# stefavpolito/EEPACC_MPC_CasADi_MATLAB

Hardware: AMD Instinct MI355X
Metric: QP steps/sec (whole node), ABMPC N=30 dense QP at batch 4096 (higher is better)
Workload: dtype f64; 1 GPU; ABMPC N=30 fp64, batch=4096 synthetic S2 ego/lead scenarios per GPU, closed loop; batch_per_gpu=4096, horizon=30, steps_per_launch=2252, parallelism=instances sharded across 1 GPU(s), no data-path collective

## Files before the change

eepacc_mpc_casadi_matlab_amd/csrc/eepacc_ab_impl.inc:

```
namespace eepacc {
namespace EEPACC_IMPL_NS {
using namespace wv;

constexpr bool kMoveBlocking = EEPACC_IMPL_MB;
constexpr bool kBaseline = EEPACC_IMPL_BL;
constexpr bool kIce = EEPACC_IMPL_ICE;
constexpr bool kTargetVeh = EEPACC_IMPL_TV;
static_assert(!kTargetVeh || kBaseline, "the target-vehicle MPC is a variant of the baseline controller");


#undef PTIC
#undef PTOC
#undef RTOC
#ifdef EEPACC_AB_TIMING
__device__ unsigned long long g_ab_prof[24];
#define PTIC(L) long long _pt = wall_clock64()
#define PTOC(L, slot) do { long long _n = wall_clock64(); (L).prof[slot] += _n - _pt; _pt = _n; } while (0)
#else
#define PTIC(L)
#define PTOC(L, slot)
#endif

constexpr double kInf = 1e300;
constexpr double kTolViol = 1e-11;
// ... 47 lines not shown

struct Lane {
    int lane, N;
    double T, tau, tau1;
    double tau_rev;
    double ba[kNumRowTypes];
    unsigned valid;
#ifdef EEPACC_AB_TIMING
    long long prof[24];
#endif
    unsigned ign;
    unsigned long long kmask;
    double lbF, lbS, lbV, lbH;
    unsigned long long code;
    double chw;
    double g0;
    double a, sh, vh, am1;
    int base;
};

__device__ __forceinline__ int code_of(const Lane& L, int t) { return (int)((L.code >> (4 * t)) & 15ull); }
__device__ __forceinline__ void set_code(Lane& L, int t, int c) {
    L.code = (L.code & ~(15ull << (4 * t))) | ((unsigned long long)c << (4 * t));
}

struct Cfg {
    int N;
    double tau_min, wF, wS, wV, wH, qH;
    int mb_len;
    const int32_t *mb_lead, *mb_end;
};

__device__ __forceinline__ double mb_reduce(const Lane& L, const Cfg& c, double x) {
    if constexpr (!kMoveBlocking) return x;
    if (c.mb_len == 0) return x;
    const int k = L.lane <= L.N ? L.lane : L.N;
    const int end = c.mb_end[k];
    const bool leader = c.mb_lead[k] == k && L.lane < L.N;
    double acc = x;
    for (int d = 1; d < c.mb_len; ++d) {
        const double y = __shfl_down(x, d, 64);
        if (L.lane + d <= end) acc += y;
    }
    return leader ? acc : 0.0;
}
__device__ __forceinline__ double mb_expand(const Lane& L, const Cfg& c, double x) {
    if constexpr (!kMoveBlocking) return x;
    if (c.mb_len == 0) return x;
    const int k = L.lane < L.N ? L.lane : 0;
    const double y = __shfl(x, c.mb_lead[k], 64);
    return L.lane < L.N ? y : x;
}

__device__ __forceinline__ double group_w(const Cfg& c, int g) {
    return g == G_F ? c.wF : (g == G_S ? c.wS : (g == G_V ? c.wV : c.wH));
}
__device__ __forceinline__ double group_lb(const Lane& L, int g) {
    return g == G_F ? L.lbF : (g == G_S ? L.lbS : (g == G_V ? L.lbV : L.lbH));
}
__device__ __forceinline__ int lane_group(const Lane& L, int t) { return L.lane == L.N ? G_NONE : group_of(t); }

__device__ __forceinline__ double row_val(const Lane& L, const Cfg& c, int t, double ba_t) {
    return row_al(t) * L.sh + row_be(t, c.tau_min, L.chw) * L.vh + row_ga(t) * L.a + row_de(t, L.lane) * L.am1 - ba_t;
}

constexpr unsigned long long kNib = 0x1111111111111111ull;
__device__ __forceinline__ unsigned long long codes_eq1(unsigned long long c) { return c & ~(c >> 1) & kNib; }
__device__ __forceinline__ unsigned long long codes_eq2(unsigned long long c) { return (c >> 1) & ~c & kNib; }
__device__ __forceinline__ constexpr unsigned long long type_range(int t0, int t1) {
    return ((t1 >= 15 ? ~0ull : ((1ull << (4 * (t1 + 1))) - 1ull)) & ~((1ull << (4 * t0)) - 1ull)) & kNib;
}
__device__ __forceinline__ int rows_below(const Lane& L, int t) {
    return __popcll(codes_eq1(L.code) & ((1ull << (4 * t)) - 1ull));
}
__device__ __forceinline__ int pivot_of(const Lane& L, int g) {
    const unsigned long long rng = kBaseline ? (g == G_F ? type_range(R_AMAX, R_VINC) : 0ull)
                                             : (g == G_F ? type_range(R_AMAX, R_VCURV)
                                                         : (g == G_S ? type_range(R_SAFE1, R_VTL) : (g == G_V ? type_range(R_VINC, R_VINC) : 0ull)));
    const unsigned long long two = codes_eq2(L.code) & rng;
    return two ? ((__ffsll((long long)two) - 1) >> 2) : -1;
}

__device__ __forceinline__ void hom_traj(const Lane& L, double x, double& sh, double& vh) {
    double xi = (L.lane < L.N) ? x : 0.0;
    vh = scan_excl(L.T * xi);
    double inc = (L.lane < L.N) ? (L.T * vh + 0.5 * L.T * L.T * xi) : 0.0;
    sh = scan_excl(inc);
}

template <int NS> constexpr bool kPackedHe = NS > 32;
template <int NS> constexpr int kHeDoubles = kPackedHe<NS> ? NS * (NS + 1) / 2 : NS * NS;

__device__ __forceinline__ double normal_at(const Lane& L, int kq, double al, double be, double ga, double de, double tau_kq) {
    double c = 0.0;
    const int j = L.lane;
    if (j < L.N) {
        if (j < kq) c = L.T * (be + al * (0.5 * L.T + tau_kq - L.tau1));
        if (j == kq) c += ga;
        if (j == kq - 1) c += de;
    }
    return c;
}

template <int NS>
__device__ __forceinline__ double adjoint(const Lane& L, const double* ws, const double* wv, const double* wa, double* tmp) {
    const int r = L.lane, N = L.N;
    const int k = N - r;
    const bool in = k >= 0;
    const double s = in ? ws[k] : 0.0, v = in ? wv[k] : 0.0;
    const double tk = in ? L.tau_rev : 0.0;
    const double WS = scan_excl(s), WV = scan_excl(v), WST = scan_excl(s * tk);
    if (in) { tmp[k] = WS; tmp[(NS + 1) + k] = WV; tmp[2 * (NS + 1) + k] = WST; }
    WSYNC();
    const int j = L.lane;
    double g = 0.0;
    if (j < N) g = wa[j] + L.T * (tmp[(NS + 1) + j] + tmp[2 * (NS + 1) + j] - (L.tau1 - 0.5 * L.T) * tmp[j]);
    WSYNC();
    return g;
}

enum Ev : int { EV_NONE = 0, EV_DROP, EV_COMPL, EV_DROPH, EV_CAP, EV_CAPIN };

template <int MMAX, int NS>
__device__ __forceinline__ void he_rank1(const Lane& L, const Cfg& c, WaveMem<MMAX, NS>& M, double* He,
                                         const double* tauv, int k, bool add) {
    const int lane = L.lane, N = L.N;
    const double chwk = bcast(L.chw, k);
    const double nk = mb_reduce(L, c, normal_at(L, k, 1.0, chwk, 0.0, 0.0, tauv[k]));
    if (lane < NS) M.yv[lane] = nk;
    WSYNC();
    const double y = he_mul<NS, kPackedHe<NS>>(He, M.yv, N, lane);
    double sy, vy;
    hom_traj(L, mb_expand(L, c, y), sy, vy);
    const double ny = bcast(sy + chwk * vy, k);
    const double kappa = add ? c.qH / (1.0 + c.qH * ny) : -c.qH / (1.0 - c.qH * ny);
    if (lane < NS) M.ub[lane] = y;
    WSYNC();
    if (lane < NS) he_sub_outer<NS, kPackedHe<NS>>(He, M.ub, kappa * y, lane);
    WSYNC();
}

template <int MMAX, int NS>
__device__ __forceinline__ void he_sync(Lane& L, const Cfg& c, WaveMem<MMAX, NS>& M, double* He, const double* tauv) {
    if constexpr (!row_live(R_HWP)) return;
    const unsigned long long want = __ballot(L.lane < L.N && code_of(L, R_HWP) == 3);
    unsigned long long diff = want ^ L.kmask;
    while (diff) {
        const int k = __ffsll((long long)diff) - 1;
        diff &= diff - 1;
        he_rank1(L, c, M, He, tauv, k, ((want >> k) & 1ull) != 0ull);
    }
    L.kmask = want;
}

template <int NS>
__device__ __forceinline__ void he_load_base(double* He, const double* __restrict__ base, int N, int lane) {
    if constexpr (kPackedHe<NS>) {
        if (lane < NS)
            for (int i = lane; i < NS; ++i) He[he_tri(i) + lane] = (i < N && lane < N) ? base[i * N + lane] : 0.0;
    } else {
#pragma unroll 4
        for (int e = lane; e < NS * NS; e += 64) {
            const int i = e / NS, j = e % NS;
            He[e] = (i < N && j < N) ? base[i * N + j] : 0.0;
        }
    }
}

template <int MMAX, int NS>
__device__ __forceinline__ int rebuild_and_factor(Lane& L, const Cfg& c, WaveMem<MMAX, NS>& M, double* Hs, const double* tauv,
                                                  const FastInfo& F) {
    const int lane = L.lane, N = L.N;
#undef RTOC
#ifdef EEPACC_AB_TIMING
    long long _q = wall_clock64();
#define RTOC(slot) do { long long _n = wall_clock64(); L.prof[slot] += _n - _q; _q = _n; } while (0)
#else
#define RTOC(slot)
#endif
    he_sync(L, c, M, Hs, tauv);
    RTOC(9);
    const int cnt = __popcll(codes_eq1(L.code));
    double basef = scan_excl((double)cnt);
    L.base = (int)(basef + 0.5);
    int m = (int)(wave_sum((double)cnt) + 0.5);
    if (m > schur_capacity<MMAX>()) return -2;
    struct PRow { double al, be, ga, de, d; };
    PRow PR[3];
#pragma unroll
    for (int gi = 0; gi < 3; ++gi) {
        const int g = G_F + gi;
        const int p = pivot_of(L, g);
        PRow r{0.0, 0.0, 0.0, 0.0, -group_lb(L, g)};
        if (p >= 0) {
            double pba = 0.0;
#pragma unroll
            for (int u = R_AMAX; u <= R_VINC; ++u) if (row_live(u) && u == p) pba = L.ba[u];
            r.al = row_al(p); r.be = row_be(p, c.tau_min, L.chw); r.ga = row_ga(p); r.de = row_de(p, lane); r.d = pba;
        }
        PR[gi] = r;
    }
    int pos = L.base;
#pragma unroll
    for (int t = 0; t < kNumRowTypes; ++t) {
        if (!row_live(t)) continue;
        int cd = code_of(L, t);
        if (cd == 1) {
            int g = lane_group(L, t);
            double al = row_al(t), be = row_be(t, c.tau_min, L.chw), ga = row_ga(t), de = row_de(t, lane);
            double d = L.ba[t];
            if (g == G_H) {
                d += L.lbH;
            } else if (g != G_NONE) {
                const int gi = group_of(t) - G_F;
                if (gi >= 0 && gi < 3) { const PRow& r = PR[gi]; al -= r.al; be -= r.be; ga -= r.ga; de -= r.de; d -= r.d; }
            }
            M.e_al[pos] = al; M.e_be[pos] = be; M.e_ga[pos] = ga; M.e_de[pos] = de;
            M.e_d[pos] = d; M.w_k[pos] = lane;
            ++pos;
        }
    }
    WSYNC();
    RTOC(10);
    if (m == 0) return 0;
    const unsigned short* rc = rc_table<MMAX>();
    if (F.fast == 1 && m == F.m_old + 1 && F.m_old > 0) {
        const int pl = rows_below(L, F.tq);
        const int p = __builtin_amdgcn_readlane(L.base + pl, __builtin_amdgcn_readfirstlane(F.kq));
        schur_insert(M.P, M.rv, rc, m, p, 1.0 / F.zz, lane);
        RTOC(12);
        return m;
    }
    if (F.fast == 2 && m == F.m_old - 1) {
        schur_remove(M.P, M.ws, rc, F.m_old, m, F.drop_pos, lane);
        RTOC(12);
        return m;
    }
    {
        const int ki = lane < m ? M.w_k[lane] : 0;
        const int kim1 = ki > 0 ? ki - 1 : 0;
        const double eal = lane < m ? M.e_al[lane] : 0.0, ebe = lane < m ? M.e_be[lane] : 0.0;
        const double ega = (lane < m && ki < N) ? M.e_ga[lane] : 0.0;
        const double ede = (lane < m && ki > 0 && ki <= N) ? M.e_de[lane] : 0.0;
        for (int j = 0; j < m; j += 2) {
            const bool two = j + 1 < m;
            const int j1 = two ? j + 1 : j;
            const int kj0 = M.w_k[j], kj1 = M.w_k[j1];
            const double c0 = mb_reduce(L, c, normal_at(L, kj0, M.e_al[j], M.e_be[j], M.e_ga[j], M.e_de[j], tauv[kj0]));
            const double c1 = mb_reduce(L, c, normal_at(L, kj1, M.e_al[j1], M.e_be[j1], M.e_ga[j1], M.e_de[j1], tauv[kj1]));
            if (lane < NS) { M.yv[lane] = c0; M.lam[lane] = c1; }
            WSYNC();
            double u0, u1;
            he_mul2<NS, kPackedHe<NS>>(Hs, M.yv, M.lam, N, lane, u0, u1);
            u0 = mb_expand(L, c, u0); u1 = mb_expand(L, c, u1);
            WSYNC();
            double su0, vu0, su1, vu1;
            hom_traj(L, u0, su0, vu0);
            hom_traj(L, u1, su1, vu1);
            const double sx = eal * __shfl(su0, ki, 64) + ebe * __shfl(vu0, ki, 64) + ega * __shfl(u0, ki, 64) + ede * __shfl(u0, kim1, 64);
            const double sy = eal * __shfl(su1, ki, 64) + ebe * __shfl(vu1, ki, 64) + ega * __shfl(u1, ki, 64) + ede * __shfl(u1, kim1, 64);
            if (lane >= j && lane < m) M.P[pidx(lane, j)] = sx;
            if (two && lane >= j + 1 && lane < m) M.P[pidx(lane, j + 1)] = sy;
        }
        WSYNC();
    }
    RTOC(11);
    const int singular = schur_invert(M.P, M.sv, M.ws, rc, m, lane);
    RTOC(12);
    if (singular) return kBaseline ? -(9 + singular) : -1;
    return m;
}

template <int MMAX, int NS>
__device__ __forceinline__ double gradient_side(const Lane& L, const Cfg& c, WaveMem<MMAX, NS>& M, int m, bool with_lam,
                                double lam_q, int kq, double qal, double qbe, double qga, double qde) {
    const int lane = L.lane, N = L.N;
    double s = 0.0, v = 0.0, a0 = 0.0, a1 = 0.0;
    if (lane < N) {
#pragma unroll
        for (int t = R_AMAX; t <= R_VINC; ++t) {
            if (row_live(t) && code_of(L, t) == 2) {
                double w = group_w(c, group_of(t));
                s += w * row_al(t); v += w * row_be(t, c.tau_min, L.chw);
                a0 += w * row_ga(t); a1 += w * row_de(t, lane);
            }
        }
    }
    if (lane < N && EEPACC_HWP_ON(L)) {
        const double wl = c.wH - c.qH * L.ba[R_HWP];
        s += wl * row_al(R_HWP); v += wl * row_be(R_HWP, c.tau_min, L.chw);
    }
// ... 7 lines not shown
        atomicAdd(&M.wv[ki], l * M.e_be[lane]);
        if (ki < N && M.e_ga[lane] != 0.0) atomicAdd(&M.wa[ki], l * M.e_ga[lane]);
        if (ki > 0 && M.e_de[lane] != 0.0) atomicAdd(&M.wa[ki - 1], l * M.e_de[lane]);
    }
    if (lam_q != 0.0 && lane == 0) {
        atomicAdd(&M.ws[kq], lam_q * qal);
        atomicAdd(&M.wv[kq], lam_q * qbe);
        if (kq < N && qga != 0.0) atomicAdd(&M.wa[kq], lam_q * qga);
        if (kq > 0 && qde != 0.0) atomicAdd(&M.wa[kq - 1], lam_q * qde);
    }
    WSYNC();
    double g = adjoint<NS>(L, M.ws, M.wv, M.wa, M.ub);
    return (lane < N) ? g + L.g0 : 0.0;
}

template <int MMAX, int NS>
__device__ __forceinline__ double direction_side(const Lane& L, WaveMem<MMAX, NS>& M, int m, int kq,
                                                 double qal, double qbe, double qga, double qde) {
    const int lane = L.lane, N = L.N;
    if (lane <= N) { M.ws[lane] = 0.0; M.wv[lane] = 0.0; M.wa[lane] = 0.0; }
    WSYNC();
    if (lane < m) {
        const int ki = M.w_k[lane];
        const double l = -M.rv[lane];
        atomicAdd(&M.ws[ki], l * M.e_al[lane]);
        atomicAdd(&M.wv[ki], l * M.e_be[lane]);
        if (ki < N && M.e_ga[lane] != 0.0) atomicAdd(&M.wa[ki], l * M.e_ga[lane]);
        if (ki > 0 && M.e_de[lane] != 0.0) atomicAdd(&M.wa[ki - 1], l * M.e_de[lane]);
    }
    if (lane == 0) {
        atomicAdd(&M.ws[kq], qal);
        atomicAdd(&M.wv[kq], qbe);
        if (kq < N && qga != 0.0) atomicAdd(&M.wa[kq], qga);
        if (kq > 0 && qde != 0.0) atomicAdd(&M.wa[kq - 1], qde);
    }
    WSYNC();
    return adjoint<NS>(L, M.ws, M.wv, M.wa, M.ub);
}

template <int MMAX, int NS>
__device__ __forceinline__ double rows_dot(const WaveMem<MMAX, NS>& M, int i, int N) {
    return rows_dot_img(M, i, N, M.ub, M.sub, M.vub);
}

template <int MMAX, int NS>
__device__ __forceinline__ void primal_from_multipliers(Lane& L, const Cfg& c, WaveMem<MMAX, NS>& M, const double* Hs, int m,
                                        double lam_q, int kq, double qal, double qbe, double qga, double qde,
                                        double& grad_total) {
    double g = gradient_side(L, c, M, m, true, lam_q, kq, qal, qbe, qga, qde);
    grad_total = g;
    g = mb_reduce(L, c, g);
    if (L.lane < NS) M.yv[L.lane] = g;
    WSYNC();
    L.a = -mb_expand(L, c, he_mul<NS, kPackedHe<NS>>(Hs, M.yv, L.N, L.lane));
    hom_traj(L, L.a, L.sh, L.vh);
    L.am1 = dpp_zero<0x138, 0xf>(L.a);
    if (L.lane < L.N) M.av[L.lane] = L.a;
    if (L.lane <= L.N) { M.shv[L.lane] = L.sh; M.vhv[L.lane] = L.vh; }
    WSYNC();
}

template <int MMAX, int NS>
__device__ __forceinline__ double refine_primal(Lane& L, const Cfg& c, WaveMem<MMAX, NS>& M, const double* Hs, int m,
                                                double lam_q, int kq, double qal, double qbe, double qga, double qde,
                                                double& grad_total, int max_rounds, double res_tol) {
    primal_from_multipliers(L, c, M, Hs, m, lam_q, kq, qal, qbe, qga, qde, grad_total);
    if (m == 0) return 0.0;
    double rel0 = 0.0;
    for (int round = 0; round < max_rounds; ++round) {
        double res = 0.0, rel = 0.0;
        if (L.lane < m) {
            res = rows_dot_img(M, L.lane, L.N, M.av, M.shv, M.vhv) - M.e_d[L.lane];
            rel = fabs(res) / (1.0 + fabs(M.e_d[L.lane]));
            M.sv[L.lane] = res;
        }
        int dummy = L.lane;
        wave_argmax(rel, dummy);
        if (round == 0) rel0 = rel;
        if (!(rel > res_tol)) break;
        WSYNC();
        if (L.lane < m) {
            double acc = 0.0;
            for (int j = 0; j < m; ++j) acc = fma(M.P[pidx(L.lane, j)], M.sv[j], acc);
            M.lam[L.lane] += acc;
        }
        WSYNC();
        primal_from_multipliers(L, c, M, Hs, m, lam_q, kq, qal, qbe, qga, qde, grad_total);
    }
    return rel0;
}

__device__ __forceinline__ double group_xi(const Lane& L, const Cfg& c, int g) {
    int p = pivot_of(L, g);
    if (p < 0) return group_lb(L, g);
    double pba = 0.0;
#pragma unroll
    for (int u = R_AMAX; u <= R_VINC; ++u) if (row_live(u) && u == p) pba = L.ba[u];
    return row_val(L, c, p, pba);
}

template <int MMAX, int NS>
__device__ __forceinline__ int warm_repair(Lane& L, const Cfg& c, const WaveMem<MMAX, NS>& M, int m, bool single, int& drop_pos) {
    const int lane = L.lane, N = L.N;
    double lmax = 0.0;
    if (lane < m) lmax = fabs(M.lam[lane]);
    lmax = wave_max(lmax);
    const double tol = kTolDual * (1.0 + lmax);
// ... 216 lines not shown
        if (F.fast == 0) L.prof[14 + why] += 1;
#endif
        if (F.fast == 0) fast_run = 0;
        const bool inc = inc_next && F.fast != 0;
        inc_next = false;
        F.m_old = m;
        m = rebuild_and_factor(L, c, M, Hs, tauv, F);
        F.fast = 0;
        PTOC(L, 0);
        if constexpr (kBaseline) {
            if (m <= -10 && warm && dep_drops < 8) {
                const int p = -m - 10;
                const int pl = M.w_k[p];
                if (lane == pl) {
                    int idx = p - L.base;
#pragma unroll
                    for (int t = 0; t < kNumRowTypes; ++t) if (row_live(t) && code_of(L, t) == 1) { if (idx == 0) set_code(L, t, 0); --idx; }
                }
                ++dep_drops;
                WSYNC();
                continue;
            }
        }
        if (m < 0) {
#ifdef EEPACC_BL_TRACE
            if (lane == 0 && (gridDim.x == 1 || g_trace_on)) printf("   factor failed (m %d, warm %d)\n", m, (int)warm);
#endif
            if (!warm) { st.status = 2; break; }
            L.code = 0ull;
            he_load_base<NS>(Hs, Hbase, N, lane);
            L.kmask = 0ull;
            WSYNC();
            warm = false;
            continue;
        }
        if (have_q) incoming_row(L, c, q);
        bool scratch = !inc;
        double rel0 = 0.0;
        if (inc && m > 0) {
            double rel = 0.0;
            if (lane < m) rel = fabs(rows_dot_img(M, lane, N, M.av, M.shv, M.vhv) - M.e_d[lane]) / (1.0 + fabs(M.e_d[lane]));
            int dummy = lane;
            wave_argmax(rel, dummy);
            rel0 = rel;
            if (rel0 > 1e-11) { scratch = true; carry_ok = false; }
#ifdef EEPACC_AB_TIMING
            L.prof[23] += scratch ? 1000 : 1;
#endif
        }
        if (scratch && m > 0) {
            double g = mb_reduce(L, c, gradient_side(L, c, M, 0, false, lam_q, q.kq, q.al, q.be, q.ga, q.de));
            if (lane < NS) M.yv[lane] = g;
            WSYNC();
            double h = mb_expand(L, c, he_mul<NS, kPackedHe<NS>>(Hs, M.yv, N, lane));
            double shh, vhh;
            hom_traj(L, h, shh, vhh);
            if (lane < N) M.ub[lane] = h;
            if (lane <= N) { M.sub[lane] = shh; M.vub[lane] = vhh; }
            WSYNC();
            solve_multipliers(M, m, lane, N);
        }
        PTOC(L, 1);
        if (scratch) {
            const double r0 = refine_primal(L, c, M, Hs, m, lam_q, q.kq, q.al, q.be, q.ga, q.de, grad_total, 3, 1e-11);
            if (r0 > rel0) rel0 = r0;
        }
        if (fast_run > 0 && rel0 > 1e-10) p_stale = true;
        PTOC(L, 2);
        if (warm && !have_q) {
            if (m > 0) {
                bool take = false;
                if constexpr (kPfAdds > 0 && !kBaseline) {
                    if (pf_left > 0) {
                        const double lam_l = (lane < m) ? M.lam[lane] : 0.0;
                        const double labs = wave_max(fabs(lam_l)), lneg = wave_max(-lam_l);
                        if (lneg > kTolDual * (1.0 + labs) && lneg <= 0.3 * labs) {
                            const int bpw = find_violation(L, c, 1e-6, best);
                            if (bpw >= 0 && (bpw & 31) < 16) {
                                q.kq = bpw >> 5; q.qcode = bpw & 31; q.is_bound = false; q.tq = q.qcode;
                                q.gq = (q.kq == N) ? G_NONE : group_of(q.qcode);
                                have_q = true; lam_q = 0.0; pf = true; take = true;
                                --pf_left; ++st.iters;
                                incoming_row(L, c, q);
#ifdef EEPACC_BL_TRACE
                                if (lane == 0 && (gridDim.x == 1 || g_trace_on)) printf("   primal first: (%d,%d) viol %.3e, worst multiplier %.3e of %.3e, m %d\n", q.kq, q.qcode, best, -lneg, labs, m);
#endif
                            }
                        }
                    }
                }
                if (!take) {
                const int rep = warm_repair(L, c, M, m, pass < kSinglePasses, F.drop_pos);
#ifdef EEPACC_BL_TRACE
                if (lane == 0 && (gridDim.x == 1 || g_trace_on)) printf("   repair pass %d: m %d -> change %d\n", pass, m, rep);
#endif
                PTOC(L, 3);
                if (rep == 2) F.fast = 2;
                WHY(1);
                if (rep) {
                    if (++pass >= kSinglePasses + 6) {
                        L.code &= ~codes_eq1(L.code);
                        he_load_base<NS>(Hs, Hbase, N, lane);
                        L.kmask = 0ull;
                        WSYNC();
                        warm = false;
                    }
                    continue;
                }
                }
            }
            if (!have_q) warm = false;
        }
        if (!have_q) {
            const int relax_every = 3 * N + 30;
            const double tolv = kTolViol * (st.iters < relax_every ? 1.0 : (st.iters < 2 * relax_every ? 10.0 : (st.iters < 3 * relax_every ? 100.0 : 1000.0)));
            int bp = find_violation(L, c, tolv > tol_floor ? tolv : tol_floor, best);
            if constexpr (kBaseline) {
                if (bp >= 0) {
                    bool again = false;
#pragma unroll
                    for (int h = 0; h < kHist; ++h) again = again || (bp == hist_bp[h] && fabs(best - hist_best[h]) <= 1e-3 * best);
                    if (again) {
                        double top = best;
#pragma unroll
                        for (int h = 0; h < kHist; ++h) if (hist_bp[h] >= 0 && hist_best[h] > top && hist_best[h] < 1e-2) top = hist_best[h];
                        if (2.0 * top < 1e-2) {
                            tol_floor = 2.0 * top;
#pragma unroll
                            for (int h = 0; h < kHist; ++h) hist_bp[h] = -1;
                            bp = find_violation(L, c, tol_floor, best);
                        }
                    }
                }
                if (bp >= 0) {
#pragma unroll
                    for (int h = kHist - 1; h > 0; --h) { hist_bp[h] = hist_bp[h - 1]; hist_best[h] = hist_best[h - 1]; }
                    hist_bp[0] = bp; hist_best[0] = best;
                }
            }
            PTOC(L, 4);
            if (bp < 0) break;
            if (++st.iters > max_iter) { st.status = 2; break; }
            q.kq = bp >> 5; q.qcode = bp & 31;
            q.is_bound = q.qcode >= 16;
            q.tq = q.is_bound ? 0 : q.qcode;
            q.gq = q.is_bound ? (q.qcode - 16) : ((q.kq == N) ? G_NONE : group_of(q.qcode));
            have_q = true; lam_q = 0.0;
            incoming_row(L, c, q);
        }
        if (++st.events > (kBaseline ? 10 : 40) * max_iter) { st.status = 2; break; }
        const int kq = q.kq;
        double viol = q.al * M.shv[kq] + q.be * M.vhv[kq] - q.d;
        if (kq < N) viol += q.ga * M.av[kq];
        if (kq > 0) viol += q.de * M.av[kq - 1];
        double cj = mb_reduce(L, c, normal_at(L, kq, q.al, q.be, q.ga, q.de, tauv[kq]));
        if (lane < NS) M.yv[lane] = cj;
        WSYNC();
        double u = mb_expand(L, c, he_mul<NS, kPackedHe<NS>>(Hs, M.yv, N, lane));
        double su, vu;
        hom_traj(L, u, su, vu);
        if (lane < N) M.ub[lane] = u;
        if (lane <= N) { M.sub[lane] = su; M.vub[lane] = vu; }
        WSYNC();
        double cu = q.al * M.sub[kq] + q.be * M.vub[kq];
        if (kq < N) cu += q.ga * M.ub[kq];
        if (kq > 0) cu += q.de * M.ub[kq - 1];
        double sr = 0.0;
        if (m > 0) {
            if (lane < m) M.sv[lane] = rows_dot(M, lane, N);
            WSYNC();
            double r = 0.0;
            if (lane < m) {
                for (int j = 0; j < m; ++j) r = fma(M.P[pidx(lane, j)], M.sv[j], r);
                M.rv[lane] = r;
                sr = M.sv[lane] * r;
            }
            WSYNC();
            sr = wave_sum(sr);
        }
        const double zz = cu - sr;
        double t2 = (zz > 1e-8 * cu) ? viol / zz : kInf;
        if (viol <= 0.0) t2 = 0.0;
        double t1 = kInf; int ev = 0x7fffffff;
        {
            double t1n = kInf, t1d = 1.0;
#define EEPACC_CAND(NUM, DEN, EVCODE) do { const double _n = (NUM), _d = (DEN); \
                if (_n * t1d < t1n * _d) { t1n = _n; t1d = _d; ev = (EVCODE); } } while (0)
            double sumLF = 0, sumLS = 0, sumLV = 0, sumRF = 0, sumRS = 0, sumRV = 0;
            int pos = L.base;
#pragma unroll
            for (int t = 0; t < kNumRowTypes; ++t) {
                if (!row_live(t)) continue;
                int cd = code_of(L, t);
                if (cd != 1) continue;
                int g2 = lane_group(L, t);
                const double l = M.lam[pos], r = M.rv[pos];
                ++pos;
                const bool blocks = !(pf && l < 0.0);
                if (g2 == G_H) {
                    if (r > 0.0) { if (blocks) EEPACC_CAND(fmax(l, 0.0), r, (EV_DROP << 16) | (lane << 5) | t); }
                    else if (r < 0.0) EEPACC_CAND(fmax(c.wH - l, 0.0), -r, (EV_COMPL << 16) | (lane << 5) | t);
                } else {
                    if (r > 0.0 && blocks) EEPACC_CAND(fmax(l, 0.0), r, (EV_DROP << 16) | (lane << 5) | t);
                    if (g2 == G_F) { sumLF += l; sumRF += r; } else if (g2 == G_S) { sumLS += l; sumRS += r; } else if (g2 == G_V) { sumLV += l; sumRV += r; }
                }
            }
            if (lane < N) {
#pragma unroll
                for (int g2 = G_F; g2 <= G_V; ++g2) {
                    double sl = g2 == G_F ? sumLF : (g2 == G_S ? sumLS : sumLV);
                    double srr = g2 == G_F ? sumRF : (g2 == G_S ? sumRS : sumRV);
// ... 31 lines not shown
                else if (q.gq == G_H) set_code(L, R_HWP, 1);
                else { int p = pivot_of(L, q.gq); set_code(L, p, 1); }
            }
            finished = true;
        } else {
            const int ek = ev >> 16, el = (ev >> 5) & 63, et = ev & 31;
            if (ek == EV_DROP) {
                const int pl = rows_below(L, et);
                F.drop_pos = __builtin_amdgcn_readlane(L.base + pl, __builtin_amdgcn_readfirstlane(el));
                F.fast = 2;
                if (lane == el) set_code(L, et, 0);
            }
            else if (ek == EV_COMPL) { if (lane == el) set_code(L, et, 3); WHY(3); }
            else if (ek == EV_DROPH) { if (lane == el) set_code(L, et, 0); finished = true; WHY(3); }
            else if (ek == EV_CAPIN) {
                if (lane == el) set_code(L, R_HWP, 3);
                finished = true; warm = true; pass = 0; WHY(3);
            }
            else if (ek == EV_CAP) {
                WHY(2);
                int fin = 0;
                if (lane == el) {
                    const int g2 = et;
                    int bestm = -1; double bl = -1e300;
                    int pos = L.base;
#pragma unroll
                    for (int t = 0; t < kNumRowTypes; ++t) {
                        if (!row_live(t)) continue;
                        if (code_of(L, t) != 1) continue;
                        const double l = M.lam[pos] - tstep * M.rv[pos];
                        ++pos;
                        if (t >= R_AMAX && t <= R_VINC && group_of(t) == g2 && l > bl) { bl = l; bestm = t; }
                    }
                    const int p = pivot_of(L, g2);
                    const bool q_row_here = (kq == el) && !q.is_bound && q.gq == g2;
                    const bool q_bound_here = (kq == el) && q.is_bound && q.gq == g2;
                    if (p < 0) {
                        if (bestm < 0) { set_code(L, q.tq, 2); fin = 1; }
                        else set_code(L, bestm, 2);
                    } else {
                        set_code(L, p, 0);
                        if (bestm >= 0) set_code(L, bestm, 2);
                        else if (q_row_here) { set_code(L, q.tq, 2); fin = 1; }
                        else if (q_bound_here) { fin = 1; }
                    }
                }
                if (__any(fin)) finished = true;
            }
        }
        if (F.fast != 0 && carry_ok) {
            const double y = mb_reduce(L, c, direction_side(L, M, m, kq, q.al, q.be, q.ga, q.de));
            if (lane < NS) M.yv[lane] = y;
            WSYNC();
            const double z = mb_expand(L, c, he_mul<NS, kPackedHe<NS>>(Hs, M.yv, N, lane));
            double sz, vz;
            hom_traj(L, z, sz, vz);
            L.a = fma(-tstep, z, L.a); L.sh = fma(-tstep, sz, L.sh); L.vh = fma(-tstep, vz, L.vh);
            L.am1 = dpp_zero<0x138, 0xf>(L.a);
            if (lane < N) M.av[lane] = L.a;
            if (lane <= N) { M.shv[lane] = L.sh; M.vhv[lane] = L.vh; }
            const double lv = (lane < m) ? fma(-tstep, M.rv[lane], M.lam[lane]) : 0.0;
            WSYNC();
            if (F.fast == 1) {
                const int pl = rows_below(L, q.tq);
                const int p = __builtin_amdgcn_readlane(L.base + pl, __builtin_amdgcn_readfirstlane(kq));
                if (lane < m && lane + 1 < MMAX) M.lam[lane < p ? lane : lane + 1] = lv;
                if (lane == 0 && p < MMAX) M.lam[p] = lam_q;
            } else {
                const int dp = F.drop_pos;
                if (lane < m && lane != dp) M.lam[lane < dp ? lane : lane - 1] = lv;
            }
            WSYNC();
            inc_next = true;
        }
        if (finished) { have_q = false; lam_q = 0.0; pf = false; q.al = q.be = q.ga = q.de = q.d = 0.0; }
        PTOC(L, 5);
    }
    if (st.status == 0 && m > 0) refine_primal(L, c, M, Hs, m, 0.0, 0, 0.0, 0.0, 0.0, 0.0, grad_total, 4, 1e-14);
    st.m = m;
    return st;
}


struct StepIn { double s, v, a_prev, t0, s_tv, v_tv, a_tv_prev; };

__device__ void force_allocation(const DevCfg& C, double s_meas, double v_meas, double a_qp,
                                 double& Fm, double& Fb, double& a_real) {
    double sn, cs;
    slope_trig(C, s_meas, sn, cs);
    double F_r = -C.zeta_a * v_meas * v_meas - C.c_r * C.m * C.g * cs - C.m * C.g * sn;
    double F_t_req = C.m * C.lambda * a_qp - F_r;
    double F_f_r_max = C.mu / C.L * (C.m * C.g * (C.L_f * cs + C.h_g * sn) +
                                     C.h_g * (C.zeta_a * v_meas * v_meas + C.lambda * C.m * a_qp));
    double F_f_tot_max = C.mu * C.m * C.g * cs;
    if (F_t_req < 0.0) {
        double F_m_min = (v_meas < C.omega_m_r / C.phi) ? -C.phi * C.T_m_max / C.eta_TF : -C.P_m_max / C.eta_TF / v_meas;
        double fm = fmax(fmax(F_t_req, F_m_min), -F_f_r_max);
        Fm = fm;
        Fb = fmax(F_t_req, -F_f_tot_max) - fm;
    } else {
        double F_m_max = (v_meas < C.omega_m_r / C.phi) ? C.phi * C.T_m_max * C.eta_TF : C.P_m_max * C.eta_TF / v_meas;
        Fm = fmin(fmin(F_t_req, F_m_max), F_f_r_max);
        Fb = 0.0;
    }
    a_real = (Fm + Fb + F_r) / C.m / C.lambda;
}

// ... 439 lines not shown
```

eepacc_mpc_casadi_matlab_amd/csrc/eepacc_kernels.hip:

```cpp
#include <hip/hip_runtime.h>
#include <math.h>
#include <stdlib.h>
#include "eepacc_device.h"
#include "eepacc_stage.h"
#include "eepacc_units.h"
#include "eepacc_schur.h"
#include "eepacc_ab.h"
#include "../../include/eepacc.h"

#define EEPACC_AB_VARIANTS(X, ...)                                       \
    X(Plain, nomb, false, false, false, false, __VA_ARGS__)              \
    X(MoveBlocking, withmb, true, false, false, false, __VA_ARGS__)      \
    X(Baseline, blc, false, true, false, false, __VA_ARGS__)             \
    X(Ice, ice, false, false, false, true, __VA_ARGS__)                  \
    X(IceMoveBlocking, icemb, true, false, false, true, __VA_ARGS__)     \
    X(TargetVehicle, tvc, false, true, true, false, __VA_ARGS__)

namespace eepacc { namespace ab_switch {
#define EEPACC_AB_SWITCHES(E, NSP, MB_, BL_, TV_, ICE_, ...) struct NSP { static constexpr bool MB = MB_, BL = BL_, TV = TV_, ICE = ICE_; };
EEPACC_AB_VARIANTS(EEPACC_AB_SWITCHES)
} }
#define EEPACC_IMPL_MB ab_switch::EEPACC_IMPL_NS::MB
#define EEPACC_IMPL_BL ab_switch::EEPACC_IMPL_NS::BL
#define EEPACC_IMPL_TV ab_switch::EEPACC_IMPL_NS::TV
#define EEPACC_IMPL_ICE ab_switch::EEPACC_IMPL_NS::ICE
#define EEPACC_IMPL_NS nomb
#include "eepacc_ab_impl.inc"
#undef EEPACC_IMPL_NS
#define EEPACC_IMPL_NS withmb
#include "eepacc_ab_impl.inc"
#undef EEPACC_IMPL_NS
#define EEPACC_IMPL_NS blc
#include "eepacc_ab_impl.inc"
#undef EEPACC_IMPL_NS
#define EEPACC_IMPL_NS ice
#include "eepacc_ab_impl.inc"
#undef EEPACC_IMPL_NS
#define EEPACC_IMPL_NS icemb
#include "eepacc_ab_impl.inc"
#undef EEPACC_IMPL_NS
#define EEPACC_IMPL_NS tvc
#include "eepacc_ab_impl.inc"
#undef EEPACC_IMPL_NS

namespace eepacc {

constexpr int kMMaxSmall = 34, kNSSmall = 32;
constexpr int kBlocksSmall = 2;
constexpr int kMMaxLarge = 66, kNSLarge = 64, kWpbLarge = 3;
constexpr int kChunkStepsDefault = nomb::kChunkStepsDefault;

#ifdef EEPACC_AB_TIMING
extern "C" int eepacc_debug_ab_prof(unsigned long long* out, int reset) {
    unsigned long long z[24] = {0};
    if (hipMemcpyFromSymbol(out, HIP_SYMBOL(nomb::g_ab_prof), sizeof(z)) != hipSuccess) return -1;
    if (reset && hipMemcpyToSymbol(HIP_SYMBOL(nomb::g_ab_prof), z, sizeof(z)) != hipSuccess) return -1;
    return 0;
}
#endif
// ... 107 lines not shown
```

eepacc_mpc_casadi_matlab_amd/csrc/eepacc_schur.h:

```cpp
#pragma once
#include <hip/hip_runtime.h>
#include <math.h>
#include "eepacc_units.h"
#include "eepacc_wave.h"

namespace eepacc {

struct SolveStats { int status, iters, events, m; };

struct FastInfo { int fast, m_old, kq, tq, drop_pos; double zz; };

struct Incoming { int kq, qcode, tq, gq; bool is_bound; double al, be, ga, de, d; };

__device__ __forceinline__ int he_tri(int i) { return i * (i + 1) / 2; }

template <int NS, bool PACKED>
__device__ __forceinline__ double he_mul(const double* Hs, const double* yv, int N, int lane) {
    double a0 = 0.0, a1 = 0.0, a2 = 0.0, a3 = 0.0;
    if constexpr (PACKED) {
        const int k = lane & (NS - 1), tk = he_tri(k);
#pragma unroll
        for (int i = 0; i < NS; i += 4) {
            a0 = fma(Hs[(i + 0) >= k ? he_tri(i + 0) + k : tk + (i + 0)], yv[i + 0], a0);
            a1 = fma(Hs[(i + 1) >= k ? he_tri(i + 1) + k : tk + (i + 1)], yv[i + 1], a1);
            a2 = fma(Hs[(i + 2) >= k ? he_tri(i + 2) + k : tk + (i + 2)], yv[i + 2], a2);
            a3 = fma(Hs[(i + 3) >= k ? he_tri(i + 3) + k : tk + (i + 3)], yv[i + 3], a3);
        }
    } else {
        const double* col = Hs + (lane & (NS - 1));
#pragma unroll
        for (int i = 0; i < NS; i += 4) {
            a0 = fma(col[(i + 0) * NS], yv[i + 0], a0);
            a1 = fma(col[(i + 1) * NS], yv[i + 1], a1);
            a2 = fma(col[(i + 2) * NS], yv[i + 2], a2);
            a3 = fma(col[(i + 3) * NS], yv[i + 3], a3);
        }
    }
    return lane < N ? (a0 + a1) + (a2 + a3) : 0.0;
}

template <int NS, bool PACKED>
__device__ __forceinline__ void he_mul2(const double* Hs, const double* y0, const double* y1, int N, int lane,
                                        double& o0, double& o1) {
    double a0 = 0.0, a1 = 0.0, b0 = 0.0, b1 = 0.0;
    const int k = lane & (NS - 1), tk = he_tri(k);
    const double* col = Hs + k;
#pragma unroll
    for (int i = 0; i < NS; i += 2) {
        double h0, h1;
        if constexpr (PACKED) {
            h0 = Hs[(i + 0) >= k ? he_tri(i + 0) + k : tk + (i + 0)];
            h1 = Hs[(i + 1) >= k ? he_tri(i + 1) + k : tk + (i + 1)];
        } else { h0 = col[(i + 0) * NS]; h1 = col[(i + 1) * NS]; }
        a0 = fma(h0, y0[i + 0], a0); b0 = fma(h0, y1[i + 0], b0);
        a1 = fma(h1, y0[i + 1], a1); b1 = fma(h1, y1[i + 1], b1);
    }
    o0 = lane < N ? a0 + a1 : 0.0;
    o1 = lane < N ? b0 + b1 : 0.0;
}

template <int NS, bool PACKED>
__device__ __forceinline__ void he_sub_outer(double* He, const double* yv, double yj, int lane) {
    if constexpr (PACKED) {
        for (int i = lane; i < NS; ++i) {
            const int e = he_tri(i) + lane;
            He[e] = fma(-yv[i], yj, He[e]);
        }
    } else {
        double* col = He + lane;
#pragma unroll
        for (int i = 0; i < NS; i += 4) {
            const double h0 = col[(i + 0) * NS], h1 = col[(i + 1) * NS], h2 = col[(i + 2) * NS], h3 = col[(i + 3) * NS];
            const double y0 = yv[i], y1 = yv[i + 1], y2 = yv[i + 2], y3 = yv[i + 3];
            col[(i + 0) * NS] = fma(-y0, yj, h0); col[(i + 1) * NS] = fma(-y1, yj, h1);
            col[(i + 2) * NS] = fma(-y2, yj, h2); col[(i + 3) * NS] = fma(-y3, yj, h3);
        }
    }
}

template <int NS>
__device__ __forceinline__ int he_invert_full(double* Hs, double* colk, int N, int lane) {
    constexpr int HALVES = 64 / NS, RPL = NS / HALVES;
    const int jcol = lane & (NS - 1), r0 = (lane & NS) / HALVES;
    double* col = Hs + jcol;
    int bad = 0;
    for (int k = 0; k < N; ++k) {
        const double d = Hs[k * NS + k];
        if (!(d > 0.0)) { bad = 1; break; }
        const double inv = 1.0 / d;
        if (lane < NS) colk[lane] = (lane < N) ? Hs[k * NS + lane] : 0.0;
        WSYNC();
        const double hkj = colk[jcol];
        const double f = hkj * inv;
        const bool piv = jcol == k;
#pragma unroll
        for (int ii = 0; ii < RPL; ++ii) {
            const int i = r0 + ii;
            const double ck = colk[i], old = col[i * NS];
            const double upd = piv ? ck * inv : fma(-ck, f, old);
            col[i * NS] = (i == k) ? (piv ? -inv : f) : upd;
        }
        WSYNC();
    }
    return bad;
}

template <int MMAX>
__host__ __device__ constexpr int schur_capacity() { return MMAX < 64 ? MMAX : 64; }

__device__ __forceinline__ void schur_insert(double* P, const double* rv, const unsigned short* rc, int m, int p,
                                             double iz, int lane) {
    const int nnz = m * (m + 1) / 2;
    for (int e0 = ((nnz - 1) >> 6) << 6; e0 >= 0; e0 -= 64) {
        const int e = e0 + lane;
        double v = 0.0;
        if (e < nnz) {
            const int code = rc[e], r = code >> 8, cc = code & 255;
            const int i = r < p ? r : r - 1, j = cc < p ? cc : cc - 1;
            if (r == p && cc == p) v = iz;
            else if (r == p) v = -rv[j] * iz;
            else if (cc == p) v = -rv[i] * iz;
            else v = P[pidx(i, j)] + rv[i] * rv[j] * iz;
        }
        WSYNC();
        if (e < nnz) P[e] = v;
        WSYNC();
    }
}

__device__ __forceinline__ void schur_remove(double* P, double* colk, const unsigned short* rc, int m_old, int m,
// ... 75 lines not shown
```

eepacc_mpc_casadi_matlab_amd/csrc/eepacc_wave.h:

```cpp
#pragma once
#include <hip/hip_runtime.h>

namespace eepacc {
namespace wv {

#define WSYNC() do { __builtin_amdgcn_fence(__ATOMIC_ACQ_REL, "wavefront"); __builtin_amdgcn_wave_barrier(); } while (0)

__device__ __forceinline__ int lane_id() { return threadIdx.x & 63; }

__device__ __forceinline__ double bcast(double x, int src) {
    const int s = __builtin_amdgcn_readfirstlane(src);
    int lo = __builtin_amdgcn_readlane(__double2loint(x), s);
    int hi = __builtin_amdgcn_readlane(__double2hiint(x), s);
    return __hiloint2double(hi, lo);
}
__device__ __forceinline__ int bcast_i(int x, int src) {
    return __builtin_amdgcn_readlane(x, __builtin_amdgcn_readfirstlane(src));
}

template <int CTRL, int ROW_MASK>
__device__ __forceinline__ double dpp_zero(double x) {
    int lo = __double2loint(x), hi = __double2hiint(x);
    lo = __builtin_amdgcn_update_dpp(0, lo, CTRL, ROW_MASK, 0xf, true);
    hi = __builtin_amdgcn_update_dpp(0, hi, CTRL, ROW_MASK, 0xf, true);
    return __hiloint2double(hi, lo);
}
template <int CTRL, int ROW_MASK>
__device__ __forceinline__ double dpp_keep(double x) {
    int lo = __double2loint(x), hi = __double2hiint(x);
    lo = __builtin_amdgcn_update_dpp(lo, lo, CTRL, ROW_MASK, 0xf, false);
    hi = __builtin_amdgcn_update_dpp(hi, hi, CTRL, ROW_MASK, 0xf, false);
    return __hiloint2double(hi, lo);
}
template <int CTRL, int ROW_MASK>
__device__ __forceinline__ double dpp_fill(double x, double fill) {
    int lo = __double2loint(x), hi = __double2hiint(x);
    lo = __builtin_amdgcn_update_dpp(__double2loint(fill), lo, CTRL, ROW_MASK, 0xf, false);
    hi = __builtin_amdgcn_update_dpp(__double2hiint(fill), hi, CTRL, ROW_MASK, 0xf, false);
    return __hiloint2double(hi, lo);
}
__device__ __forceinline__ double read_lane63(double x) {
    int lo = __builtin_amdgcn_readlane(__double2loint(x), 63);
    int hi = __builtin_amdgcn_readlane(__double2hiint(x), 63);
    return __hiloint2double(hi, lo);
}
__device__ __forceinline__ double lane_prev(double x) { return dpp_zero<0x138, 0xf>(x); }
__device__ __forceinline__ double lane_next(double x) { return dpp_zero<0x130, 0xf>(x); }

__device__ __forceinline__ double scan_incl(double x) {
    x += dpp_zero<0x111, 0xf>(x);
    x += dpp_zero<0x112, 0xf>(x);
    x += dpp_zero<0x114, 0xf>(x);
    x += dpp_zero<0x118, 0xf>(x);
    x += dpp_zero<0x142, 0xa>(x);
    x += dpp_zero<0x143, 0xc>(x);
    return x;
}
__device__ __forceinline__ double wave_sum(double x) { return read_lane63(scan_incl(x)); }
__device__ __forceinline__ double scan_excl(double x) { return dpp_zero<0x138, 0xf>(scan_incl(x)); }
__device__ __forceinline__ double scan_prod_excl(double x) {
    x *= dpp_fill<0x111, 0xf>(x, 1.0);
    x *= dpp_fill<0x112, 0xf>(x, 1.0);
    x *= dpp_fill<0x114, 0xf>(x, 1.0);
    x *= dpp_fill<0x118, 0xf>(x, 1.0);
    x *= dpp_fill<0x142, 0xa>(x, 1.0);
    x *= dpp_fill<0x143, 0xc>(x, 1.0);
    return dpp_fill<0x138, 0xf>(x, 1.0);
}
__device__ __forceinline__ double wave_max(double x) {
    x = fmax(x, dpp_keep<0x111, 0xf>(x));
    x = fmax(x, dpp_keep<0x112, 0xf>(x));
    x = fmax(x, dpp_keep<0x114, 0xf>(x));
    x = fmax(x, dpp_keep<0x118, 0xf>(x));
    x = fmax(x, dpp_keep<0x142, 0xa>(x));
    x = fmax(x, dpp_keep<0x143, 0xc>(x));
    return read_lane63(x);
}
__device__ __forceinline__ void wave_argmax(double& v, int& p) {
    const double best = wave_max(v);
    const unsigned long long mask = __ballot(v == best);
    const int src = mask ? (__ffsll((long long)mask) - 1) : 0;
    p = __builtin_amdgcn_readlane(p, src);
    v = best;
}
__device__ __forceinline__ void wave_argmin(double& v, int& p) {
    double nv = -v;
    wave_argmax(nv, p);
    v = -nv;
}

}
}
```

Before: 17.30 million QP steps/s.

## Split Hessian matvec and Schur columns across both wave halves for NS=32

For the unpacked 32-wide Hessian, the matvec and rank-1 update now split each column's rows between the two 32-lane halves of the wave and combine the partial sums with a permlane32 swap. Previously only 32 lanes did the work. The Schur column build now computes four columns per iteration, two per half-wave, using half-wave scans and shuffles. This is meant to use the idle upper lanes and cut serial LDS loop length, at the cost of extra cross-half data movement and more complex indexing.

```diff
diff --git a/eepacc_mpc_casadi_matlab_amd/csrc/eepacc_ab_cols.h b/eepacc_mpc_casadi_matlab_amd/csrc/eepacc_ab_cols.h
--- /dev/null
+++ b/eepacc_mpc_casadi_matlab_amd/csrc/eepacc_ab_cols.h
@@ -0,0 +1,72 @@
+#pragma once
+#include "eepacc_schur.h"
+
+namespace eepacc {
+
+__device__ __forceinline__ double ab_normal_at_half(int j, int N, double T, double tau1, int kq, double al, double be,
+                                                    double ga, double de, double tau_kq) {
+    double c = 0.0;
+    if (j < N) {
+        if (j < kq) c = T * (be + al * (0.5 * T + tau_kq - tau1));
+        if (j == kq) c += ga;
+        if (j == kq - 1) c += de;
+    }
+    return c;
+}
+
+__device__ __forceinline__ void ab_hom_traj_half(int j, int N, double T, double x, double& sh1, double& vh1) {
+    const int lane = wv::lane_id();
+    double xi = (j < N) ? x : 0.0;
+    vh1 = wv::scan_incl_half(T * xi);
+    double vh = wv::dpp_zero<0x138, 0xf>(vh1);
+    vh = lane == 32 ? 0.0 : vh;
+    double inc = (j < N) ? (T * vh + 0.5 * T * T * xi) : 0.0;
+    sh1 = wv::scan_incl_half(inc);
+}
+
+template <int NS, class Mem, class Reduce, class Expand>
+__device__ __forceinline__ void ab_schur_columns4(Mem& M, const double* Hs, const double* tauv, int m, int N, int lane,
+                                                  double T, double tau1, Reduce reduce, Expand expand) {
+    static_assert(NS == 32, "two horizons per wave");
+    const int hl = lane & (NS - 1), up = (lane >> 5) & 1;
+    double* y0 = up ? M.sv : M.yv;
+    double* y1 = up ? M.rv : M.lam;
+    const int ki = lane < m ? M.w_k[lane] : 0;
+    const int kim1 = ki > 0 ? ki - 1 : 0;
+    const int kiu = ki < NS ? ki : NS - 1;
+    const double eal = lane < m ? M.e_al[lane] : 0.0, ebe = lane < m ? M.e_be[lane] : 0.0;
+    const double ega = (lane < m && ki < N) ? M.e_ga[lane] : 0.0;
+    const double ede = (lane < m && ki > 0 && ki <= N) ? M.e_de[lane] : 0.0;
+    for (int j = 0; j < m; j += 4) {
+        const int ja = min(j + 2 * up, m - 1), jb = min(j + 2 * up + 1, m - 1);
+        const int kj0 = M.w_k[ja], kj1 = M.w_k[jb];
+        const double c0 = reduce(ab_normal_at_half(hl, N, T, tau1, kj0, M.e_al[ja], M.e_be[ja], M.e_ga[ja], M.e_de[ja], tauv[kj0]));
+        const double c1 = reduce(ab_normal_at_half(hl, N, T, tau1, kj1, M.e_al[jb], M.e_be[jb], M.e_ga[jb], M.e_de[jb], tauv[kj1]));
+        y0[hl] = c0; y1[hl] = c1;
+        WSYNC();
+        double u0, u1;
+        he_mul2<NS, false>(Hs, y0, y1, N, hl, u0, u1);
+        u0 = expand(u0); u1 = expand(u1);
+        WSYNC();
+        double su0, vu0, su1, vu1;
+        ab_hom_traj_half(hl, N, T, u0, su0, vu0);
+        ab_hom_traj_half(hl, N, T, u1, su1, vu1);
+#pragma unroll
+        for (int h = 0; h < 2; ++h) {
+            const int sk = kiu + 32 * h, sk1 = kim1 + 32 * h;
+            double s0 = __shfl(su0, sk1, 64), v0 = __shfl(vu0, sk1, 64), a0 = __shfl(u0, sk, 64);
+            double s1 = __shfl(su1, sk1, 64), v1 = __shfl(vu1, sk1, 64), a1 = __shfl(u1, sk, 64);
+            const double d0 = __shfl(u0, sk1, 64), d1 = __shfl(u1, sk1, 64);
+            s0 = ki > 0 ? s0 : 0.0; v0 = ki > 0 ? v0 : 0.0; a0 = ki < N ? a0 : 0.0;
+            s1 = ki > 0 ? s1 : 0.0; v1 = ki > 0 ? v1 : 0.0; a1 = ki < N ? a1 : 0.0;
+            const double sx = eal * s0 + ebe * v0 + ega * a0 + ede * d0;
+            const double sy = eal * s1 + ebe * v1 + ega * a1 + ede * d1;
+            const int col = j + 2 * h;
+            if (col < m && lane >= col && lane < m) M.P[pidx(lane, col)] = sx;
+            if (col + 1 < m && lane >= col + 1 && lane < m) M.P[pidx(lane, col + 1)] = sy;
+        }
+    }
+    WSYNC();
+}
+
+}
diff --git a/eepacc_mpc_casadi_matlab_amd/csrc/eepacc_ab_impl.inc b/eepacc_mpc_casadi_matlab_amd/csrc/eepacc_ab_impl.inc
--- a/eepacc_mpc_casadi_matlab_amd/csrc/eepacc_ab_impl.inc
+++ b/eepacc_mpc_casadi_matlab_amd/csrc/eepacc_ab_impl.inc
@@ -123,6 +123,29 @@
     return L.lane < L.N ? y : x;
 }
 
+__device__ __forceinline__ double mb_reduce_half(const Lane& L, const Cfg& c, double x) {
+    if constexpr (!kMoveBlocking) return x;
+    if (c.mb_len == 0) return x;
+    const int hl = L.lane & 31;
+    const int k = hl <= L.N ? hl : L.N;
+    const int end = c.mb_end[k];
+    const bool leader = c.mb_lead[k] == k && hl < L.N;
+    double acc = x;
+    for (int d = 1; d < c.mb_len; ++d) {
+        const double y = __shfl_down(x, d, 64);
+        if (hl + d <= end) acc += y;
+    }
+    return leader ? acc : 0.0;
+}
+__device__ __forceinline__ double mb_expand_half(const Lane& L, const Cfg& c, double x) {
+    if constexpr (!kMoveBlocking) return x;
+    if (c.mb_len == 0) return x;
+    const int hl = L.lane & 31;
+    const int k = hl < L.N ? hl : 0;
+    const double y = __shfl(x, c.mb_lead[k] + (L.lane & 32), 64);
+    return hl < L.N ? y : x;
+}
+
 __device__ __forceinline__ double group_w(const Cfg& c, int g) {
     return g == G_F ? c.wF : (g == G_S ? c.wS : (g == G_V ? c.wV : c.wH));
 }
@@ -161,6 +184,12 @@
 
 template <int NS> constexpr bool kPackedHe = NS > 32;
 template <int NS> constexpr int kHeDoubles = kPackedHe<NS> ? NS * (NS + 1) / 2 : NS * NS;
+
+template <int NS>
+__device__ __forceinline__ double he_apply(const double* Hs, const double* yv, int N, int lane) {
+    if constexpr (kPackedHe<NS>) return he_mul<NS, true>(Hs, yv, N, lane);
+    else return he_mul_halves<NS>(Hs, yv, N, lane);
+}
 
 __device__ __forceinline__ double normal_at(const Lane& L, int kq, double al, double be, double ga, double de, double tau_kq) {
     double c = 0.0;
@@ -200,14 +229,18 @@
     const double nk = mb_reduce(L, c, normal_at(L, k, 1.0, chwk, 0.0, 0.0, tauv[k]));
     if (lane < NS) M.yv[lane] = nk;
     WSYNC();
-    const double y = he_mul<NS, kPackedHe<NS>>(He, M.yv, N, lane);
+    const double y = he_apply<NS>(He, M.yv, N, lane);
     double sy, vy;
     hom_traj(L, mb_expand(L, c, y), sy, vy);
     const double ny = bcast(sy + chwk * vy, k);
     const double kappa = add ? c.qH / (1.0 + c.qH * ny) : -c.qH / (1.0 - c.qH * ny);
     if (lane < NS) M.ub[lane] = y;
     WSYNC();
-    if (lane < NS) he_sub_outer<NS, kPackedHe<NS>>(He, M.ub, kappa * y, lane);
+    if constexpr (kPackedHe<NS>) {
+        if (lane < NS) he_sub_outer<NS, true>(He, M.ub, kappa * y, lane);
+    } else {
+        he_sub_outer_halves<NS>(He, M.ub, kappa * M.ub[lane & (NS - 1)], lane);
+    }
     WSYNC();
 }
 
@@ -307,7 +340,10 @@
         RTOC(12);
         return m;
     }
-    {
+    if constexpr (!kPackedHe<NS>) {
+        ab_schur_columns4<NS>(M, Hs, tauv, m, N, lane, half_lo(L.T), half_lo(L.tau1),
+                              [&](double x) { return mb_reduce_half(L, c, x); }, [&](double x) { return mb_expand_half(L, c, x); });
+    } else {
         const int ki = lane < m ? M.w_k[lane] : 0;
         const int kim1 = ki > 0 ? ki - 1 : 0;
         const double eal = lane < m ? M.e_al[lane] : 0.0, ebe = lane < m ? M.e_be[lane] : 0.0;
@@ -421,7 +457,7 @@
     g = mb_reduce(L, c, g);
     if (L.lane < NS) M.yv[L.lane] = g;
     WSYNC();
-    L.a = -mb_expand(L, c, he_mul<NS, kPackedHe<NS>>(Hs, M.yv, L.N, L.lane));
+    L.a = -mb_expand(L, c, he_apply<NS>(Hs, M.yv, L.N, L.lane));
     hom_traj(L, L.a, L.sh, L.vh);
     L.am1 = dpp_zero<0x138, 0xf>(L.a);
     if (L.lane < L.N) M.av[L.lane] = L.a;
@@ -744,7 +780,7 @@
             double g = mb_reduce(L, c, gradient_side(L, c, M, 0, false, lam_q, q.kq, q.al, q.be, q.ga, q.de));
             if (lane < NS) M.yv[lane] = g;
             WSYNC();
-            double h = mb_expand(L, c, he_mul<NS, kPackedHe<NS>>(Hs, M.yv, N, lane));
+            double h = mb_expand(L, c, he_apply<NS>(Hs, M.yv, N, lane));
             double shh, vhh;
             hom_traj(L, h, shh, vhh);
             if (lane < N) M.ub[lane] = h;
@@ -848,7 +884,7 @@
         double cj = mb_reduce(L, c, normal_at(L, kq, q.al, q.be, q.ga, q.de, tauv[kq]));
         if (lane < NS) M.yv[lane] = cj;
         WSYNC();
-        double u = mb_expand(L, c, he_mul<NS, kPackedHe<NS>>(Hs, M.yv, N, lane));
+        double u = mb_expand(L, c, he_apply<NS>(Hs, M.yv, N, lane));
         double su, vu;
         hom_traj(L, u, su, vu);
         if (lane < N) M.ub[lane] = u;
@@ -986,7 +1022,7 @@
             const double y = mb_reduce(L, c, direction_side(L, M, m, kq, q.al, q.be, q.ga, q.de));
             if (lane < NS) M.yv[lane] = y;
             WSYNC();
-            const double z = mb_expand(L, c, he_mul<NS, kPackedHe<NS>>(Hs, M.yv, N, lane));
+            const double z = mb_expand(L, c, he_apply<NS>(Hs, M.yv, N, lane));
             double sz, vz;
             hom_traj(L, z, sz, vz);
             L.a = fma(-tstep, z, L.a); L.sh = fma(-tstep, sz, L.sh); L.vh = fma(-tstep, vz, L.vh);
diff --git a/eepacc_mpc_casadi_matlab_amd/csrc/eepacc_kernels.hip b/eepacc_mpc_casadi_matlab_amd/csrc/eepacc_kernels.hip
--- a/eepacc_mpc_casadi_matlab_amd/csrc/eepacc_kernels.hip
+++ b/eepacc_mpc_casadi_matlab_amd/csrc/eepacc_kernels.hip
@@ -5,6 +5,7 @@
 #include "eepacc_stage.h"
 #include "eepacc_units.h"
 #include "eepacc_schur.h"
+#include "eepacc_ab_cols.h"
 #include "eepacc_ab.h"
 #include "../../include/eepacc.h"
 
diff --git a/eepacc_mpc_casadi_matlab_amd/csrc/eepacc_schur.h b/eepacc_mpc_casadi_matlab_amd/csrc/eepacc_schur.h
--- a/eepacc_mpc_casadi_matlab_amd/csrc/eepacc_schur.h
+++ b/eepacc_mpc_casadi_matlab_amd/csrc/eepacc_schur.h
@@ -76,6 +76,42 @@
             col[(i + 2) * NS] = fma(-y2, yj, h2); col[(i + 3) * NS] = fma(-y3, yj, h3);
         }
     }
+}
+
+
+template <int NS>
+__device__ __forceinline__ void he_sub_outer_halves(double* He, const double* yv, double yj, int lane) {
+    static_assert(NS == 32, "two lanes per column");
+    constexpr int RPL = NS / 2;
+    const int r0 = (lane & NS) / 2;
+    double* col = He + r0 * NS + (lane & (NS - 1));
+    const double* y = yv + r0;
+#pragma unroll
+    for (int i = 0; i < RPL; i += 4) {
+        const double h0 = col[(i + 0) * NS], h1 = col[(i + 1) * NS], h2 = col[(i + 2) * NS], h3 = col[(i + 3) * NS];
+        const double y0 = y[i], y1 = y[i + 1], y2 = y[i + 2], y3 = y[i + 3];
+        col[(i + 0) * NS] = fma(-y0, yj, h0); col[(i + 1) * NS] = fma(-y1, yj, h1);
+        col[(i + 2) * NS] = fma(-y2, yj, h2); col[(i + 3) * NS] = fma(-y3, yj, h3);
+    }
+}
+
+template <int NS>
+__device__ __forceinline__ double he_mul_halves(const double* Hs, const double* yv, int N, int lane) {
+    static_assert(NS == 32, "two lanes per column");
+    constexpr int RPL = NS / 2;
+    const int r0 = (lane & NS) / 2;
+    const double* col = Hs + r0 * NS + (lane & (NS - 1));
+    const double* y = yv + r0;
+    double a0 = 0.0, a1 = 0.0, a2 = 0.0, a3 = 0.0;
+#pragma unroll
+    for (int i = 0; i < RPL; i += 4) {
+        a0 = fma(col[(i + 0) * NS], y[i + 0], a0);
+        a1 = fma(col[(i + 1) * NS], y[i + 1], a1);
+        a2 = fma(col[(i + 2) * NS], y[i + 2], a2);
+        a3 = fma(col[(i + 3) * NS], y[i + 3], a3);
+    }
+    const double s = wv::half_sum((a0 + a1) + (a2 + a3));
+    return lane < N ? s : 0.0;
 }
 
 template <int NS>
diff --git a/eepacc_mpc_casadi_matlab_amd/csrc/eepacc_wave.h b/eepacc_mpc_casadi_matlab_amd/csrc/eepacc_wave.h
--- a/eepacc_mpc_casadi_matlab_amd/csrc/eepacc_wave.h
+++ b/eepacc_mpc_casadi_matlab_amd/csrc/eepacc_wave.h
@@ -58,6 +58,27 @@
 }
 __device__ __forceinline__ double wave_sum(double x) { return read_lane63(scan_incl(x)); }
 __device__ __forceinline__ double scan_excl(double x) { return dpp_zero<0x138, 0xf>(scan_incl(x)); }
+__device__ __forceinline__ double scan_incl_half(double x) {
+    x += dpp_zero<0x111, 0xf>(x);
+    x += dpp_zero<0x112, 0xf>(x);
+    x += dpp_zero<0x114, 0xf>(x);
+    x += dpp_zero<0x118, 0xf>(x);
+    x += dpp_zero<0x142, 0xa>(x);
+    return x;
+}
+__device__ __forceinline__ double scan_excl_half(double x) {
+    x = dpp_zero<0x138, 0xf>(scan_incl_half(x));
+    return lane_id() == 32 ? 0.0 : x;
+}
+__device__ __forceinline__ void half_pair(double x, double& lo, double& hi) {
+    const unsigned xl = (unsigned)__double2loint(x), xh = (unsigned)__double2hiint(x);
+    const auto a = __builtin_amdgcn_permlane32_swap(xl, xl, false, false);
+    const auto b = __builtin_amdgcn_permlane32_swap(xh, xh, false, false);
+    lo = __hiloint2double((int)b[0], (int)a[0]);
+    hi = __hiloint2double((int)b[1], (int)a[1]);
+}
+__device__ __forceinline__ double half_lo(double x) { double lo, hi; half_pair(x, lo, hi); return lo; }
+__device__ __forceinline__ double half_sum(double x) { double lo, hi; half_pair(x, lo, hi); return lo + hi; }
 __device__ __forceinline__ double scan_prod_excl(double x) {
     x *= dpp_fill<0x111, 0xf>(x, 1.0);
     x *= dpp_fill<0x112, 0xf>(x, 1.0);
```

Result: faster. 19.09 million QP steps/s (median of 6 runs) (+10.3%).
